# yaricom/Plastic-UNet

Hardware: AMD Instinct MI355X
Metric: training images/sec (128x128, bs=32 per GPU) (higher is better)
Workload: dtype f32; 1 GPU; C2: UNetp depth 5 base_ch 64, oja rule, 1x128x128, fwd+BCE+bwd+Adam; global_batch=32, per_gpu_batch=32, img=128, parallelism=single, step_launch=eager

## Files before the change

### plastic-unet_amd/csrc/wgrad.hip

```cpp
#include "common.h"
#include <type_traits>

#ifndef PU_NO_ILV
#define PU_NO_ILV 0
#endif
#ifndef PU_WW_ABL
#define PU_WW_ABL 0
#endif

namespace pu {

typedef float f32x4 __attribute__((ext_vector_type(4)));
typedef float f32x16 __attribute__((ext_vector_type(16)));

constexpr int WG_BM = 16;

struct WgradParams {
    int M, N, Nr, K, Kc, C, c0, c1;
    int Hi, Wi, Ho, Wo, kw, stride, pad;
    const float* P;
    const float* src0;
    const float* src1;
    int bias_mode;
    float* slab;
// ... 914 lines not shown
        sub(k, std::integral_constant<int, 1>{});
        sub(k, std::integral_constant<int, 2>{});
        sub(k, std::integral_constant<int, 3>{});
    }
    asm volatile("s_waitcnt vmcnt(0) lgkmcnt(0)" ::: "memory");

    float* slab = p.slab + (long long)z * p.Nr * p.Kcp;
    if (p.bias_mode == 1 && cx == 0) {
        wg_f32x2* red = reinterpret_cast<wg_f32x2*>(lg0);
        red[tid] = bsum;
        __syncthreads();
        if (tid < 32) {
            wg_f32x2 v = red[tid];
            for (int r = 1; r < 16; ++r) v += red[r * 32 + tid];
            slab[(long long)(ny * 64 + 2 * tid) * p.Kcp + p.K] = v[0];
            slab[(long long)(ny * 64 + 2 * tid + 1) * p.Kcp + p.K] = v[1];
        }
        __syncthreads();
    }

    const float sj1 = wj ? -1.f : 1.f;
    float* xs = reinterpret_cast<float*>(wc ? lx1 : lx0) + (wn * 2 + wj) * 24 * 64;
    const float* xrd = reinterpret_cast<const float*>(wc ? lx1 : lx0) + (wn * 2 + (1 - wj)) * 24 * 64;
    const int lr = lane & 31, lh = lane >> 5;
    const int n = ny * 64 + wn * 32 + lr;
#pragma unroll
    for (int r = 0; r < 3; ++r) {
        float mine[2][3][4], other[2][3][4];
#pragma unroll
        for (int q = 0; q < 4; ++q)
#pragma unroll
            for (int ee = 0; ee < 4; ++ee) {
                const int idx = 4 * q + ee;
                float R[2];
#pragma unroll
                for (int jj = 0; jj < 2; ++jj) {
                    const float m0 = acc[0 * 2 + jj][idx], m1 = acc[1 * 2 + jj][idx];
                    const float m2 = acc[2 * 2 + jj][idx], m3 = -acc[3 * 2 + jj][idx];
                    float v = r == 0 ? m0 + 0.5f * (m1 + m2) : r == 1 ? 0.5f * (m1 - m2) : 0.5f * (m1 + m2) + m3;
                    R[jj] = jj == 1 ? sj1 * v : v;
                }
                float P[3];
                if (wj == 0) {
                    P[0] = R[0] + 0.5f * R[1];
                    P[1] = 0.5f * R[1];
                    P[2] = 0.5f * R[1];
                } else {
                    P[0] = 0.5f * R[0];
                    P[1] = -0.5f * R[0];
                    P[2] = 0.5f * R[0] + R[1];
                }
                const bool keep = (q >> 1) == wj;
#pragma unroll
                for (int s = 0; s < 3; ++s) {
                    if (keep) mine[q & 1][s][ee] = P[s];
                    else other[q & 1][s][ee] = P[s];
                }
            }
#pragma unroll
        for (int qh = 0; qh < 2; ++qh)
#pragma unroll
            for (int s = 0; s < 3; ++s)
#pragma unroll
                for (int ee = 0; ee < 4; ++ee) xs[((qh * 3 + s) * 4 + ee) * 64 + lane] = other[qh][s][ee];
        __syncthreads();
#pragma unroll
        for (int qh = 0; qh < 2; ++qh)
#pragma unroll
            for (int s = 0; s < 3; ++s) {
                f32x4 v;
#pragma unroll
                for (int ee = 0; ee < 4; ++ee) {
                    const float o = xrd[((qh * 3 + s) * 4 + ee) * 64 + lane];
                    v[ee] = wj == 0 ? mine[qh][s][ee] + o : o + mine[qh][s][ee];
                }
                const int q = 2 * wj + qh;
                const int k = (3 * r + s) * p.C + c_lo + wc * 32 + 8 * q + 4 * lh;
                *reinterpret_cast<f32x4*>(slab + (long long)n * p.Kcp + k) = v;
            }
        __syncthreads();
    }
}

constexpr int SWS_TH = 16, SWS_TW = 64;

template <int N, bool BF16ROWS = false>
__global__ __launch_bounds__(256) void wgrad_stem_kernel(const WgradParams p) {
    constexpr int L = N / 4, PG = 256 / L;
    constexpr int HH = SWS_TH + 2, HW = SWS_TW + 2;
    constexpr int RED = PG * 10 * N;
    __shared__ __attribute__((aligned(16))) float smem[RED > HH * HW ? RED : HH * HW];
    const int tid = threadIdx.x;
    const int lane_c = tid % L, grp = tid / L;
    float acc[10][4];
#pragma unroll
    for (int k = 0; k < 10; ++k)
#pragma unroll
        for (int e = 0; e < 4; ++e) acc[k][e] = 0.f;
    const int ntiles = p.batch * p.tiles_h * p.tiles_w;
    for (int t = blockIdx.x; t < ntiles; t += gridDim.x) {
        const int txi = t % p.tiles_w;
        const int tyi = (t / p.tiles_w) % p.tiles_h;
        const int b = t / (p.tiles_w * p.tiles_h);
        const int y0 = tyi * SWS_TH - 1, x0 = txi * SWS_TW - 1;
        const long long img = (long long)b * p.Hi * p.Wi;
        __syncthreads();
        for (int e = tid; e < HH * HW; e += 256) {
            const int hy = e / HW, hx = e - hy * HW;
            const int gy = y0 + hy, gx = x0 + hx;
            smem[e] = ((unsigned)gy < (unsigned)p.Hi && (unsigned)gx < (unsigned)p.Wi)
                          ? p.src0[img + (long long)gy * p.Wi + gx] : 0.f;
        }
        __syncthreads();
        static_assert((SWS_TH * SWS_TW) % (4 * PG) == 0, "stem wgrad pass");
        for (int q0 = grp; q0 < SWS_TH * SWS_TW; q0 += 4 * PG) {
            f32x4 dzs[4];
            bool ok[4];
            int hb[4];
#pragma unroll
            for (int u = 0; u < 4; ++u) {
                const int q = q0 + u * PG;
                const int row = q / SWS_TW, col = q - row * SWS_TW;
                const int oy = tyi * SWS_TH + row, ox = txi * SWS_TW + col;
                ok[u] = oy < p.Ho && ox < p.Wo;
                hb[u] = row * HW + col;
                const long long m = ok[u] ? ((long long)b * p.Ho + oy) * p.Wo + ox : 0;
                if constexpr (BF16ROWS) {
                    typedef __bf16 bf16x4_t __attribute__((ext_vector_type(4)));
                    const bf16x4_t zb = *reinterpret_cast<const bf16x4_t*>(reinterpret_cast<const __bf16*>(p.P) + m * N + 4 * lane_c);
#pragma unroll
                    for (int e = 0; e < 4; ++e) dzs[u][e] = (float)zb[e];
                } else {
                    dzs[u] = *reinterpret_cast<const f32x4*>(p.P + m * N + 4 * lane_c);
                }
            }
#pragma unroll
            for (int u = 0; u < 4; ++u) {
                if (!ok[u]) continue;
                const f32x4 dz = dzs[u];
#pragma unroll
                for (int t9 = 0; t9 < 9; ++t9) {
                    const float a = smem[hb[u] + (t9 / 3) * HW + t9 % 3];
#pragma unroll
                    for (int e = 0; e < 4; ++e) acc[t9][e] = fmaf(a, dz[e], acc[t9][e]);
                }
#pragma unroll
                for (int e = 0; e < 4; ++e) acc[9][e] += dz[e];
            }
        }
    }
    __syncthreads();
#pragma unroll
    for (int k = 0; k < 10; ++k)
#pragma unroll
        for (int e = 0; e < 4; ++e) smem[(grp * 10 + k) * N + 4 * lane_c + e] = acc[k][e];
    __syncthreads();
    float* slab = p.slab + (long long)blockIdx.x * p.Nr * p.Kcp;
    for (int idx = tid; idx < 10 * N; idx += 256) {
        const int k = idx / N, n = idx - k * N;
        float v = 0.f;
        for (int g = 0; g < PG; ++g) v += smem[(g * 10 + k) * N + n];
        slab[(long long)n * p.Kcp + k] = v;
    }
}

template <int C, int N>
// ... 296 lines not shown
__global__ __launch_bounds__(256) void wgrad_sum_splits4_kernel(const float* __restrict__ slab, int splits,
                                                                long long total, int G, double* __restrict__ part) {
    const long long idx = 4 * (blockIdx.x * (long long)blockDim.x + threadIdx.x);
    if (idx >= total) return;
    const int g = blockIdx.y;
    const f64x4 s = sum_chains<8>(reinterpret_cast<const f32x4*>(slab + (long long)g * total + idx),
                                  (splits - g + G - 1) / G, G * (total >> 2));
    double* o = part + (long long)g * total + idx;
#pragma unroll
    for (int e = 0; e < 4; ++e) o[e] = s[e];
}

template <typename T>
__global__ __launch_bounds__(256) void wgrad_finish4_kernel(const T* __restrict__ part, int G, int Nr, int Kc, int N,
                                                            int K, int C, int kh, int kw, int bias_mode,
                                                            float* __restrict__ dw, float* __restrict__ db,
                                                            int accumulate) {
    typedef T t4 __attribute__((ext_vector_type(4)));
    const long long total = (long long)Nr * Kc;
    const long long nq = total >> 2;
    const long long q = blockIdx.x * (long long)blockDim.x + threadIdx.x;
    if (q < nq) {
        const long long idx = 4 * q;
        const int n = int(idx / Kc);
        const int k0 = int(idx - (long long)n * Kc);
        if (n >= N) return;
        const f64x4 s = sum_chains<8>(reinterpret_cast<const t4*>(part + idx), G, nq);
#pragma unroll
        for (int e = 0; e < 4; ++e) store_oihw(n, k0 + e, (float)s[e], K, C, kh, kw, bias_mode, dw, db, accumulate);
    } else if (bias_mode == 2 && q < nq + C) {
        const int c = int(q - nq);
        const int J = kh * kw * G;
        const T* bp = part + (long long)N * Kc + c;
        auto at = [&](int j) {
            const int t = j / G, gg = j - t * G;
            return (double)bp[(long long)gg * total + t * C];
        };
        double s[4] = {0.0, 0.0, 0.0, 0.0};
        int j = 0;
        for (; j + 7 < J; j += 8) {
            double v[8];
#pragma unroll
            for (int u = 0; u < 8; ++u) v[u] = at(j + u);
#pragma unroll
            for (int u = 0; u < 8; ++u) s[u & 3] += v[u];
        }
        for (; j < J; ++j) s[0] += at(j);
        const float v = (float)((s[0] + s[1]) + (s[2] + s[3]));
        db[c] = accumulate ? db[c] + v : v;
    }
}

template <typename T>
__global__ __launch_bounds__(576) void wgrad_finish_t_kernel(const T* __restrict__ part, int G, int Nr, int Kc, int K,
                                                              int C, int taps, int bias_mode, float* __restrict__ dw,
                                                              float* __restrict__ db, int accumulate) {
    __shared__ float tr[256 * 9];
    typedef T t4 __attribute__((ext_vector_type(4)));
    const long long total = (long long)Nr * Kc;
    const int n = blockIdx.y;
    const int c0 = blockIdx.x * 256;
    const int tap = threadIdx.x >> 6, cq = (threadIdx.x & 63) * 4;
    const int cn = min(256, C - c0);
    if (cq < cn) {
        const long long idx = (long long)n * Kc + tap * C + c0 + cq;
        const f64x4 s = sum_chains<4>(reinterpret_cast<const t4*>(part) + (idx >> 2), G, total >> 2);
#pragma unroll
        for (int e = 0; e < 4; ++e) tr[(cq + e) * taps + tap] = (float)s[e];
    }
    if (bias_mode == 1 && blockIdx.x == 0 && threadIdx.x == 0) {
        const float v = (float)sum_chains<4>(part + (long long)n * Kc + K, G, total);
        db[n] = accumulate ? db[n] + v : v;
    }
    __syncthreads();
    float* o = dw + ((long long)n * C + c0) * taps;
    const int run = cn * taps;
    for (int i = threadIdx.x * 4; i < run; i += blockDim.x * 4) {
        f32x4 v = {tr[i], tr[i + 1], tr[i + 2], tr[i + 3]};
        if (accumulate) v += *reinterpret_cast<const f32x4*>(o + i);
        *reinterpret_cast<f32x4*>(o + i) = v;
    }
}

struct WgradPlan {
    int BN, BK, splits, mps, Nr, Kc, Kcp, M, K, C, G, gx, gy;
    bool qvec, dma, small, halo, stem;
    bool wino = false;
    bool pw = false;
    int tiles = 0, tps = 0;
    int nt = 1;
    int tiles_w, tiles_h;
    size_t slab_bytes() const { return (size_t)splits * Nr * Kcp * sizeof(float); }
    size_t part_bytes() const { return G > 1 ? (size_t)G * Nr * Kcp * sizeof(double) : 0; }
    size_t ws_bytes() const { return ((slab_bytes() + 255) / 256) * 256 + part_bytes(); }
};

static bool stem_wgrad_ok(const pu_wgrad_args* a) {
    return a->c0 == 1 && a->c1 == 0 && (a->n == 8 || a->n == 16 || a->n == 32 || a->n == 64) && a->kh == 3 && a->kw == 3 && a->stride == 1 &&
           a->pad == 1 && a->in_h == a->out_h && a->in_w == a->out_w && a->bias_mode == 1 &&
           ((uintptr_t)a->rows & 15) == 0;
}

static bool pw_wgrad_ok(const pu_wgrad_args* a) {
    const int C = a->c0, N = a->n;
    return a->c1 == 0 && a->kh == 1 && a->kw == 1 && a->stride == 1 && a->pad == 0 && a->in_h == a->out_h &&
           a->in_w == a->out_w && a->bias_mode != 2 && (C == 3 || C == 4) && (N == 4 || N == 8 || N == 16) &&
           (((uintptr_t)a->rows & 15) == 0) && (C % 4 || ((uintptr_t)a->src0 & 15) == 0);
}

static bool small_wgrad_ok(const pu_wgrad_args* a) {
    const int C = a->c0 + a->c1;
    return (C == 1 || C == 4 || C == 8 || C == 12 || C == 16) &&
           (a->n == 4 || a->n == 8 || a->n == 16) && a->kh == 3 && a->kw == 3 && a->stride == 1 && a->pad == 1 &&
           a->in_h == a->out_h && a->in_w == a->out_w && a->bias_mode != 2 &&
           (C == 1 || (a->c0 % 4 == 0 && a->c1 % 4 == 0));
}

static void plan_groups(WgradPlan* pl) {
    const long long total = (long long)pl->Nr * pl->Kcp;
    int G = (int)ceil_div(262144LL, total);
    const int by_len = ceil_div(pl->splits, 8);
    if (G > by_len) G = by_len;
    if (G > 16) G = 16;
    pl->G = G < 1 ? 1 : G;
}

static int plan_dims(const pu_wgrad_args* a, WgradPlan* pl, const char* who) {
    const long long M = (long long)a->batch * a->out_h * a->out_w;
    PU_REQUIRE(M < (1LL << 31), "%s: too many pixels", who);
    pl->M = (int)M;
    pl->C = a->c0 + a->c1;
    pl->K = a->kh * a->kw * pl->C;
    pl->Nr = a->n + (a->bias_mode == 2 ? 1 : 0);
    pl->Kc = pl->K + (a->bias_mode == 1 ? 1 : 0);
    pl->Kcp = (pl->Kc + 3) / 4 * 4;
    return PU_OK;
}

static void plan_halo(const pu_wgrad_args* a, WgradPlan* pl) {
    pl->halo = true;
    pl->nt = a->n % 128 == 0 ? 2 : 1;
    pl->BN = 64 * pl->nt;
    pl->BK = 9 * 64;
    pl->gx = pl->C / 64;
    pl->gy = a->n / pl->BN;
    int splits = (pl->nt == 2 ? 256 : 512) / (pl->gx * pl->gy);
    const int stages = pl->M / 16;
    if (splits > stages) splits = stages;
    if (splits < 1) splits = 1;
    pl->mps = ceil_div(stages, splits) * 16;
    pl->splits = ceil_div(pl->M, pl->mps);
    plan_groups(pl);
}

static bool wino_wgrad_ok(const pu_wgrad_args* a, const WgradPlan* pl) {
    static const bool on = [] {
        const char* e = getenv("PU_WINO_WGRAD");
        return !(e && e[0] == '0');
    }();
    if (!on || a->math != 1 || !pl->qvec) return false;
    if (a->kh != 3 || a->kw != 3 || a->stride != 1 || a->pad != 1) return false;
    if (a->in_h != a->out_h || a->in_w != a->out_w || (a->out_h & 1) || (a->out_w & 1)) return false;
    if (a->c0 % 64 || a->c1 % 64 || a->n % 64 || a->bias_mode == 2) return false;
    const long long px = (long long)a->batch * a->in_h * a->in_w + a->in_w + 1;
    if (px * (a->c0 > a->c1 ? a->c0 : a->c1) * 4 >= (1LL << 31)) return false;
    if ((long long)a->batch * a->out_h * a->out_w * a->n * 4 >= (1LL << 31)) return false;
    return (((uintptr_t)a->rows | (uintptr_t)a->src0 | (uintptr_t)a->src1) & 7) == 0;
}

static int plan_wgrad(const pu_wgrad_args* a, WgradPlan* pl) {
    PU_REQUIRE(a && a->batch > 0 && a->out_h > 0 && a->out_w > 0 && a->in_h > 0 && a->in_w > 0, "pu_wgrad: bad grid");
    PU_REQUIRE(a->kh > 0 && a->kw > 0 && a->stride > 0 && a->pad >= 0, "pu_wgrad: bad taps");
    PU_REQUIRE(a->rows && a->n > 0 && a->src0 && a->c0 > 0 && (a->c1 == 0 || a->src1), "pu_wgrad: operands");
    PU_REQUIRE(a->n % 4 == 0, "pu_wgrad: n (%d) must be a multiple of 4", a->n);
    PU_REQUIRE(a->bias_mode >= 0 && a->bias_mode <= 2, "pu_wgrad: bias_mode");
    PU_REQUIRE(a->bias_mode == 0 || a->dbias, "pu_wgrad: dbias missing");
    PU_REQUIRE(a->dweight, "pu_wgrad: dweight missing");
    PU_REQUIRE(a->math >= 0 && a->math <= 2, "pu_wgrad: math %d", a->math);
    PU_REQUIRE(a->math != 2 || stem_wgrad_ok(a), "pu_wgrad: math 2 (bf16 rows) is the single-channel stem only");
    if (int st = plan_dims(a, pl, "pu_wgrad")) return st;
    const long long M = pl->M;
    pl->qvec = (a->c0 % 4 == 0) && (a->c1 % 4 == 0);
    pl->small = small_wgrad_ok(a);
    pl->stem = stem_wgrad_ok(a);
    pl->pw = pw_wgrad_ok(a);
    pl->halo = false;
    if (pl->qvec) {
        PU_REQUIRE(((uintptr_t)a->src0 & 15) == 0 && ((uintptr_t)a->src1 & 15) == 0, "pu_wgrad: sources must be 16-byte aligned");
    }
    PU_REQUIRE(((uintptr_t)a->rows & 15) == 0, "pu_wgrad: rows must be 16-byte aligned");
    pl->dma = pl->qvec;
    if (pl->pw) {
        pl->splits = (int)(M / 256 < 1024 ? (M + 255) / 256 : 1024);
        pl->mps = (int)ceil_div(M, (long long)pl->splits);
        pl->splits = (int)ceil_div(M, (long long)pl->mps);
        pl->BN = a->n; pl->BK = pl->K; pl->gx = pl->gy = 1; pl->dma = false;
        pl->tiles_w = pl->tiles_h = 0;
        plan_groups(pl);
        return PU_OK;
    }
    if (pl->small || pl->stem) {
        pl->tiles_w = ceil_div(a->out_w, pl->stem ? SWS_TW : SW_TW);
        pl->tiles_h = ceil_div(a->out_h, pl->stem ? SWS_TH : SW_TH);
        const long long ntiles = (long long)a->batch * pl->tiles_w * pl->tiles_h;
        pl->splits = (int)(ntiles < 1024 ? ntiles : 1024);
        pl->BN = a->n; pl->BK = pl->K; pl->gx = pl->gy = 1; pl->mps = 0; pl->dma = false;
        plan_groups(pl);
        return PU_OK;
    }
    const int ext_n = pl->dma ? a->n : pl->Nr;
    const int ext_k = pl->dma ? pl->K : pl->Kc;
    int occ;
    if (ext_k <= 64) { pl->BN = 64; pl->BK = 64; occ = pl->dma ? 6 : 7; }
    else if (ext_n <= 64 && !pl->dma) { pl->BN = 64; pl->BK = 256; occ = 3; }
    else if (ext_n <= 32 && a->math == 1) { pl->BN = 32; pl->BK = 128; occ = 4; }
    else if (ext_n <= 64) {
        const bool b192 = ceil_div(ext_k, 192) * 192 < ceil_div(ext_k, 128) * 128;
        pl->BN = 64; pl->BK = b192 ? 192 : 128; occ = b192 ? 3 : 4;
    }
    else { pl->BN = 128; pl->BK = 128; occ = pl->dma ? 3 : 4; }
    if (a->math == 1 && pl->dma && pl->BN == 128 &&
        ceil_div(ext_k, 256) * 256 <= ceil_div(ext_k, 128) * 128) {
        pl->BK = 256;
        occ = 2;
    }
    pl->halo = false;
    if (wino_wgrad_ok(a, pl)) {
        pl->wino = true;
        pl->BN = 64;
        pl->BK = 9 * 64;
        pl->gx = pl->C / 64;
        pl->gy = a->n / 64;
        pl->tiles = a->batch * (a->out_h / 2) * (a->out_w / 2);
        const int stages = ceil_div(pl->tiles, 16);
        int splits = 256 / (pl->gx * pl->gy);
        if (splits > stages) splits = stages;
        if (splits < 1) splits = 1;
        pl->tps = ceil_div(stages, splits) * 16;
        pl->splits = ceil_div(pl->tiles, pl->tps);
        pl->mps = pl->tps * 4;
        plan_groups(pl);
        return PU_OK;
    }
    if (a->math == 1 && pl->dma && a->kh == 3 && a->kw == 3 && a->stride == 1 && a->pad == 1 &&
        a->in_h == a->out_h && a->in_w == a->out_w && a->out_w % 16 == 0 && a->c0 % 64 == 0 && a->c1 % 64 == 0 &&
        a->n % 64 == 0 && a->bias_mode != 2 && (long long)a->batch * a->in_h * a->in_w * (pl->C) < (1LL << 31)) {
        plan_halo(a, pl);
        return PU_OK;
    }
    pl->gx = ceil_div(ext_k, pl->BK);
    pl->gy = ceil_div(ext_n, pl->BN);
    const int tiles = pl->gx * pl->gy;
    const int slots = 256 * occ;
    int splits = slots / tiles;
    int max_splits = ceil_div(M, 256);
    if (splits > max_splits) splits = max_splits;
    if (splits < 1) splits = 1;
    int mps = ceil_div(ceil_div(M, splits), WG_BM) * WG_BM;
    pl->mps = mps;
    pl->splits = ceil_div(M, mps);
    plan_groups(pl);
    return PU_OK;
}

typedef __bf16 wbf16x8 __attribute__((ext_vector_type(8)));
__device__ __attribute__((aligned(16))) __bf16 g_wg_zero_b16[8];

constexpr int WB_ROWS = 32;
constexpr int WB_W = 128;


struct WgradBf16Params {
    int M, N, K, Kcp, Nr, C, c0, c1;
    int Hi, Wi, Ho, Wo, kw, stride, pad;
    const __bf16* P;
    const __bf16* src0;
    const __bf16* src1;
    int bias_mode;
    float* slab;
    int mps, gx, gy;
    FastDiv dWo, dHo, dC, dKw;
};

__global__ __launch_bounds__(256) void wgrad_bf16_kernel(const WgradBf16Params p) {
    constexpr int NBUF = 3;
    constexpr int LD = WB_ROWS * WB_W * 2 / 1024 / 4;
    constexpr int G = 2 * LD;
    constexpr int IMG = WB_ROWS * WB_W;
    constexpr int STAGE = 2 * IMG;
    __shared__ __attribute__((aligned(16))) __bf16 lds[NBUF * STAGE];

    const int tid = threadIdx.x;
    const int lane = tid & 63;
    const int wave = __builtin_amdgcn_readfirstlane(tid >> 6);
    const int wn = wave & 1, wk = wave >> 1;
    const int lr = lane & 31, lh = lane >> 5;
    const int tile = xcd_remap(blockIdx.x, gridDim.x);
    const int tx = tile % p.gx;
    const int tyz = tile / p.gx;
    const int ty = tyz % p.gy;
    const int tz = tyz / p.gy;
    const int n_blk = ty * WB_W;
    const int k_blk = tx * WB_W;
    const int m_begin = tz * p.mps;
    const int m_end = min(p.M, m_begin + p.mps);

    const int lrow = lane >> 4;
    int p_col[LD], q_r[LD], q_s[LD], q_cs[LD];
    const __bf16* q_ptr[LD];
// ... 283 lines not shown
        asm volatile("s_waitcnt lgkmcnt(0)" ::: "memory");
        __builtin_amdgcn_s_barrier();
        asm volatile("" ::: "memory");
    }
    int g = 0;
    for (; g + 1 < NG; g += 2) {
        group(g, std::integral_constant<int, 0>{});
        group(g + 1, std::integral_constant<int, 1>{});
    }
    if (g < NG) group(g, std::integral_constant<int, 0>{});

    float* slab = p.slab + (long long)tz * p.Nr * p.Kcp;
    if (bias_blk) {
        f32x4* red = reinterpret_cast<f32x4*>(lds);
        red[tid] = bsum;
        __syncthreads();
        if (tid < 16 * NT) {
            f32x4 v = red[tid];
            for (int r = 1; r < 16; ++r) v += red[r * 16 * NT + tid];
#pragma unroll
            for (int e = 0; e < 4; ++e) slab[(long long)(ty * 64 * NT + tid * 4 + e) * p.Kcp + p.K] = v[e];
        }
    }
    const int lr = lane & 31, lh = lane >> 5;
    const int n = ty * 64 * NT + nt * 64 + nj * 32 + lr;
#pragma unroll
    for (int t9 = 0; t9 < 9; ++t9) {
#pragma unroll
        for (int q = 0; q < 4; ++q) {
            const int k = t9 * p.C + c_lo + ci * 32 + 8 * q + 4 * lh;
            f32x4 v;
#pragma unroll
            for (int e = 0; e < 4; ++e) v[e] = acc[t9][4 * q + e];
            *reinterpret_cast<f32x4*>(slab + (long long)n * p.Kcp + k) = v;
        }
    }
}

constexpr int WR_E = 16, WR_S = 64;
__global__ __launch_bounds__(256) void wgrad_reduce_wide_kernel(const float* __restrict__ slab, int splits,
                                                                 long long total, int N, int Kcp, int K, int C,
                                                                 int kh, int kw, int bias_mode, float* __restrict__ dw,
                                                                 float* __restrict__ db, int accumulate) {
    __shared__ double part[WR_S][WR_E];
    const int quad = threadIdx.x & 3, sl = threadIdx.x >> 2;
    const long long idx0 = (long long)blockIdx.x * WR_E + 4 * quad;
    f64x4 a = {};
    if (idx0 < total)
        a = sum_chains<4>(reinterpret_cast<const f32x4*>(slab + (long long)sl * total + idx0),
                          (splits - sl + WR_S - 1) / WR_S, WR_S * (total >> 2));
#pragma unroll
    for (int e = 0; e < 4; ++e) part[sl][4 * quad + e] = a[e];
    __syncthreads();
    if (threadIdx.x >= WR_E) return;
    const long long idx = (long long)blockIdx.x * WR_E + threadIdx.x;
    if (idx >= total) return;
    double sum = 0.0;
    for (int l = 0; l < WR_S; ++l) sum += part[l][threadIdx.x];
    const int n = (int)(idx / Kcp), k = (int)(idx - (long long)n * Kcp);
    if (n >= N) return;
    store_oihw(n, k, (float)sum, K, C, kh, kw, bias_mode, dw, db, accumulate);
}

template <typename T>
static void launch_finisher(bool transposed, const T* part, int count, const WgradPlan& pl, const pu_wgrad_args* a,
                            hipStream_t s) {
    const int taps = a->kh * a->kw;
    if (transposed) {
        hipLaunchKernelGGL(wgrad_finish_t_kernel<T>, dim3((unsigned)ceil_div(pl.C, 256), (unsigned)a->n),
                           dim3((unsigned)(64 * taps)), 0, s, part, count, pl.Nr, pl.Kcp, pl.K, pl.C, taps, a->bias_mode,
                           a->dweight, a->dbias, a->accumulate);
        return;
    }
    const long long threads = (long long)pl.Nr * pl.Kcp / 4 + (a->bias_mode == 2 ? pl.C : 0);
    hipLaunchKernelGGL(wgrad_finish4_kernel<T>, dim3((unsigned)((threads + 255) / 256)), dim3(256), 0, s, part, count,
                       pl.Nr, pl.Kcp, a->n, pl.K, pl.C, a->kh, a->kw, a->bias_mode, a->dweight, a->dbias, a->accumulate);
}

constexpr long long WR_WIDE_MAX = 16384;

static int wgrad_reduce(const WgradPlan& pl, const pu_wgrad_args* a, void* workspace, hipStream_t s) {
    const long long total = (long long)pl.Nr * pl.Kcp;
    const float* slab = (const float*)workspace;
    if ((pl.small || pl.stem || pl.pw || (!pl.wino && total <= WR_WIDE_MAX)) && a->bias_mode != 2) {
        hipLaunchKernelGGL(wgrad_reduce_wide_kernel, dim3((unsigned)ceil_div(total, (long long)WR_E)), dim3(256), 0, s,
                           slab, pl.splits, total, a->n, pl.Kcp, pl.K, pl.C, a->kh, a->kw, a->bias_mode, a->dweight,
                           a->dbias, a->accumulate);
        return check_launch("pu_wgrad (reduce)");
    }
    const bool transposed = a->bias_mode != 2 && a->kh * a->kw <= 9 && pl.C % 4 == 0 && ((uintptr_t)a->dweight & 15) == 0;
    if (pl.G > 1) {
        double* part = (double*)((char*)workspace + ((pl.slab_bytes() + 255) / 256) * 256);
        hipLaunchKernelGGL(wgrad_sum_splits4_kernel, dim3((unsigned)((total / 4 + 255) / 256), pl.G), dim3(256), 0, s,
                           slab, pl.splits, total, pl.G, part);
        launch_finisher(transposed, (const double*)part, pl.G, pl, a, s);
    } else {
        launch_finisher(transposed, slab, pl.splits, pl, a, s);
    }
    return check_launch("pu_wgrad (reduce)");
}

static int plan_wgrad_bf16(const pu_wgrad_args* a, WgradPlan* pl) {
    PU_REQUIRE(a && a->batch > 0 && a->out_h > 0 && a->out_w > 0 && a->in_h > 0 && a->in_w > 0, "pu_wgrad_bf16: bad grid");
    PU_REQUIRE(a->kh > 0 && a->kw > 0 && a->stride > 0 && a->pad >= 0, "pu_wgrad_bf16: bad taps");
    PU_REQUIRE(a->rows && a->n > 0 && a->src0 && a->c0 > 0 && (a->c1 == 0 || a->src1), "pu_wgrad_bf16: operands");
    PU_REQUIRE(a->n % 8 == 0 && a->c0 % 8 == 0 && a->c1 % 8 == 0,
               "pu_wgrad_bf16: n (%d) and channel counts (%d, %d) must be multiples of 8", a->n, a->c0, a->c1);
    PU_REQUIRE(a->bias_mode >= 0 && a->bias_mode <= 2 && (a->bias_mode == 0 || a->dbias) && a->dweight, "pu_wgrad_bf16: outputs");
    PU_REQUIRE((((uintptr_t)a->rows | (uintptr_t)a->src0 | (uintptr_t)a->src1) & 15) == 0, "pu_wgrad_bf16: 16-byte alignment");
    if (int st = plan_dims(a, pl, "pu_wgrad_bf16")) return st;
    const long long M = pl->M;
    pl->qvec = true; pl->dma = true; pl->small = false; pl->stem = false;
    pl->halo = false;
    if (a->kh == 3 && a->kw == 3 && a->stride == 1 && a->pad == 1 && a->in_h == a->out_h &&
        a->in_w == a->out_w && a->out_w % 16 == 0 && a->c0 % 64 == 0 && a->c1 % 64 == 0 && a->n % 64 == 0 &&
        a->bias_mode != 2 && M * pl->C < (1LL << 31)) {
        plan_halo(a, pl);
        return PU_OK;
    }
    pl->BN = WB_W; pl->BK = WB_W;
    pl->gx = ceil_div(pl->K, WB_W);
    pl->gy = ceil_div(a->n, WB_W);
    const int tiles = pl->gx * pl->gy;
    int splits = 768 / tiles;
    const int max_splits = ceil_div(M, 512);
    if (splits > max_splits) splits = max_splits;
    if (splits < 1) splits = 1;
    pl->mps = ceil_div(ceil_div(M, splits), WB_ROWS) * WB_ROWS;
    pl->splits = ceil_div(M, pl->mps);
    plan_groups(pl);
    return PU_OK;
}

}

using namespace pu;

extern "C" size_t pu_wgrad_workspace_bytes(const pu_wgrad_args* a) {
    WgradPlan pl;
    if (plan_wgrad(a, &pl) != PU_OK) return 0;
    return pl.ws_bytes();
}

extern "C" int pu_wgrad_tile(const pu_wgrad_args* a, int* bn, int* bk, int* qvec, int* splits) {
    WgradPlan pl;
    int st = plan_wgrad(a, &pl);
    if (st != PU_OK) return st;
    if (bn) *bn = pl.BN;
    if (bk) *bk = pl.BK;
    if (qvec) *qvec = pl.pw ? 6 : pl.wino ? 5 : pl.stem ? 4 : pl.small ? 2 : pl.halo ? 3 : (pl.qvec ? 1 : 0);
    if (splits) *splits = pl.splits;
    return PU_OK;
}

extern "C" int pu_wgrad(const pu_wgrad_args* a, void* workspace, size_t ws_bytes, void* stream) {
    return pu_wgrad_phase(a, workspace, ws_bytes, 3, stream);
}

extern "C" int pu_wgrad_phase(const pu_wgrad_args* a, void* workspace, size_t ws_bytes, int phase, void* stream) {
    PU_REQUIRE(phase >= 1 && phase <= 3, "pu_wgrad_phase: phase %d", phase);
    WgradPlan pl;
    int st = plan_wgrad(a, &pl);
    if (st != PU_OK) return st;
    const size_t need = pl.ws_bytes();
    if (!workspace || ws_bytes < need)
        return fail(PU_ERR_WORKSPACE, "pu_wgrad: workspace %zu < %zu bytes", ws_bytes, need);

    WgradParams p;
    p.M = pl.M; p.N = a->n; p.Nr = pl.Nr; p.K = pl.K; p.Kc = pl.Kc; p.Kcp = pl.Kcp; p.C = pl.C; p.c0 = a->c0; p.c1 = a->c1;
    p.Hi = a->in_h; p.Wi = a->in_w; p.Ho = a->out_h; p.Wo = a->out_w;
    p.kw = a->kw; p.stride = a->stride; p.pad = a->pad;
    p.P = a->rows; p.src0 = a->src0; p.src1 = a->src1; p.bias_mode = a->bias_mode;
    p.slab = (float*)workspace; p.mps = pl.mps;
    p.dWo = make_fastdiv(a->out_w); p.dHo = make_fastdiv(a->out_h);
    p.dC = make_fastdiv(pl.C); p.dKw = make_fastdiv(a->kw);

    hipStream_t s = as_stream(stream);
    p.gx = pl.gx;
    p.gy = pl.gy;
    p.batch = a->batch; p.tiles_w = pl.tiles_w; p.tiles_h = pl.tiles_h;
    if (pl.stem && (phase & 1) && a->math == 2) {
        if (a->n == 64) hipLaunchKernelGGL((wgrad_stem_kernel<64, true>), dim3(pl.splits), dim3(256), 0, s, p);
        else if (a->n == 32) hipLaunchKernelGGL((wgrad_stem_kernel<32, true>), dim3(pl.splits), dim3(256), 0, s, p);
        else if (a->n == 16) hipLaunchKernelGGL((wgrad_stem_kernel<16, true>), dim3(pl.splits), dim3(256), 0, s, p);
        else hipLaunchKernelGGL((wgrad_stem_kernel<8, true>), dim3(pl.splits), dim3(256), 0, s, p);
        st = check_launch("pu_wgrad (stem, bf16 rows)");
        if (st != PU_OK) return st;
        phase &= ~1;
    }
    if (pl.stem && (phase & 1)) {
        if (a->n == 64) hipLaunchKernelGGL(wgrad_stem_kernel<64>, dim3(pl.splits), dim3(256), 0, s, p);
        else if (a->n == 32) hipLaunchKernelGGL(wgrad_stem_kernel<32>, dim3(pl.splits), dim3(256), 0, s, p);
        else if (a->n == 16) hipLaunchKernelGGL(wgrad_stem_kernel<16>, dim3(pl.splits), dim3(256), 0, s, p);
        else hipLaunchKernelGGL(wgrad_stem_kernel<8>, dim3(pl.splits), dim3(256), 0, s, p);
        st = check_launch("pu_wgrad (stem)");
        if (st != PU_OK) return st;
        phase &= ~1;
    }
    if (pl.pw && (phase & 1)) {
        const int C = pl.C, N = a->n;
        const dim3 sg(pl.splits);
#define PU_PW(C_, N_) if (C == C_ && N == N_) hipLaunchKernelGGL((wgrad_pw_kernel<C_, N_>), sg, dim3(256), 0, s, p)
        PU_PW(3, 4); else PU_PW(3, 8); else PU_PW(3, 16); else PU_PW(4, 4); else PU_PW(4, 8); else PU_PW(4, 16);
#undef PU_PW
        st = check_launch("pu_wgrad (pointwise)");
        if (st != PU_OK) return st;
        phase &= ~1;
    }
    if (pl.small && (phase & 1)) {
        const int C = pl.C, N = a->n;
        const dim3 sg(pl.splits);
#define PU_SW(C_, N_) if (C == C_ && N == N_) hipLaunchKernelGGL((wgrad_small_kernel<C_, N_>), sg, dim3(256), 0, s, p)
        PU_SW(1, 4); else PU_SW(1, 8); else PU_SW(1, 16); else PU_SW(4, 4); else PU_SW(4, 8); else PU_SW(4, 16);
        else PU_SW(8, 4); else PU_SW(8, 8); else PU_SW(8, 16); else PU_SW(12, 4); else PU_SW(12, 8);
        else PU_SW(12, 16); else PU_SW(16, 4); else PU_SW(16, 8); else PU_SW(16, 16);
#undef PU_SW
        st = check_launch("pu_wgrad (small-channel)");
        if (st != PU_OK) return st;
        phase &= ~1;
    }
    dim3 grid(p.gx * p.gy * pl.splits);
    const bool fq = a->stride == 1 && a->in_h == a->out_h && a->in_w == a->out_w && a->out_w >= 4;
    if (phase & 1) {
#define PU_WG_DMA(BN_, BK_, WN_, WK_)                                                                    \
    do {                                                                                                     \
        if (a->math == 1 && fq) hipLaunchKernelGGL((wgrad_dma_kernel<BN_, BK_, WN_, WK_, 3, true, 4, true>), grid, dim3(256), 0, s, p); \
        else if (a->math == 1) hipLaunchKernelGGL((wgrad_dma_kernel<BN_, BK_, WN_, WK_, 3, true>), grid, dim3(256), 0, s, p); \
        else hipLaunchKernelGGL((wgrad_dma_kernel<BN_, BK_, WN_, WK_, 3, false>), grid, dim3(256), 0, s, p); \
    } while (0)
#define PU_WG_REG(BN_, BK_, WN_, WK_, Q_) hipLaunchKernelGGL((wgrad_kernel<BN_, BK_, WN_, WK_, Q_>), grid, dim3(256), 0, s, p)
        if (pl.wino) {
            WinoWgradParams ww;
            ww.p = p;
            ww.tiles = pl.tiles;
            ww.tps = pl.tps;
            ww.dTw = make_fastdiv(a->out_w / 2);
            ww.dTh = make_fastdiv(a->out_h / 2);
            const long long px = (long long)a->batch * a->in_h * a->in_w + a->in_w + 1;
            ww.x0_bytes = (unsigned)(px * a->c0 * 4);
            ww.x1_bytes = (unsigned)(px * a->c1 * 4);
            ww.p_bytes = (unsigned)((long long)pl.M * a->n * 4);
            hipLaunchKernelGGL(wgrad_wino_x6_kernel, grid, dim3(512), 0, s, ww);
        } else if (pl.halo) {
            if (pl.nt == 2) hipLaunchKernelGGL(wgrad_halo_x6_kernel<2>, grid, dim3(512), 0, s, p);
            else hipLaunchKernelGGL(wgrad_halo_x6_kernel<1>, grid, dim3(256), 0, s, p);
        } else if (pl.dma) {
            if (pl.BK == 64) PU_WG_DMA(64, 64, 2, 2);
            else if (pl.BN == 64 && pl.BK == 128) PU_WG_DMA(64, 128, 2, 2);
            else if (pl.BN == 32) PU_WG_DMA(32, 128, 1, 4);
            else if (pl.BK == 192) PU_WG_DMA(64, 192, 2, 2);
            else if (pl.BK == 256 && fq) hipLaunchKernelGGL((wgrad_dma_kernel<128, 256, 2, 2, 3, true, 4, true>), grid, dim3(256), 0, s, p);
            else if (pl.BK == 256) hipLaunchKernelGGL((wgrad_dma_kernel<128, 256, 2, 2, 3, true>), grid, dim3(256), 0, s, p);
            else PU_WG_DMA(128, 128, 2, 2);
        } else if (pl.qvec) {
            if (pl.BK == 64) PU_WG_REG(64, 64, 2, 2, true);
            else if (pl.BK == 256) PU_WG_REG(64, 256, 1, 4, true);
            else PU_WG_REG(128, 128, 2, 2, true);
        } else {
            if (pl.BK == 64) PU_WG_REG(64, 64, 2, 2, false);
            else if (pl.BK == 256) PU_WG_REG(64, 256, 1, 4, false);
            else PU_WG_REG(128, 128, 2, 2, false);
        }
#undef PU_WG_DMA
#undef PU_WG_REG
        st = check_launch("pu_wgrad (gemm)");
        if (st != PU_OK) return st;
    }
    if (!(phase & 2)) return PU_OK;
    return wgrad_reduce(pl, a, workspace, s);
}

extern "C" size_t pu_wgrad_bf16_workspace_bytes(const pu_wgrad_args* a) {
    WgradPlan pl;
    if (plan_wgrad_bf16(a, &pl) != PU_OK) return 0;
    return pl.ws_bytes();
}

extern "C" int pu_wgrad_bf16_phase(const pu_wgrad_args* a, void* workspace, size_t ws_bytes, int phase, void* stream) {
    PU_REQUIRE(phase >= 1 && phase <= 3, "pu_wgrad_bf16_phase: phase %d", phase);
    WgradPlan pl;
    int st = plan_wgrad_bf16(a, &pl);
    if (st != PU_OK) return st;
    const size_t need = pl.ws_bytes();
    if (!workspace || ws_bytes < need)
        return fail(PU_ERR_WORKSPACE, "pu_wgrad_bf16: workspace %zu < %zu bytes", ws_bytes, need);
    hipStream_t s = as_stream(stream);
    if (phase & 1) {
        WgradBf16Params p;
        p.M = pl.M; p.N = a->n; p.K = pl.K; p.Kcp = pl.Kcp; p.Nr = pl.Nr; p.C = pl.C; p.c0 = a->c0; p.c1 = a->c1;
        p.Hi = a->in_h; p.Wi = a->in_w; p.Ho = a->out_h; p.Wo = a->out_w;
        p.kw = a->kw; p.stride = a->stride; p.pad = a->pad;
        p.P = (const __bf16*)a->rows; p.src0 = (const __bf16*)a->src0; p.src1 = (const __bf16*)a->src1;
        p.bias_mode = a->bias_mode;
        p.slab = (float*)workspace; p.mps = pl.mps; p.gx = pl.gx; p.gy = pl.gy;
        p.dWo = make_fastdiv(a->out_w); p.dHo = make_fastdiv(a->out_h);
        p.dC = make_fastdiv(pl.C); p.dKw = make_fastdiv(a->kw);
        if (pl.halo && pl.nt == 2) hipLaunchKernelGGL(wgrad_halo_bf16_kernel<2>, dim3(pl.gx * pl.gy * pl.splits), dim3(512), 0, s, p);
        else if (pl.halo) hipLaunchKernelGGL(wgrad_halo_bf16_kernel<1>, dim3(pl.gx * pl.gy * pl.splits), dim3(256), 0, s, p);
        else hipLaunchKernelGGL(wgrad_bf16_kernel, dim3(pl.gx * pl.gy * pl.splits), dim3(256), 0, s, p);
        st = check_launch("pu_wgrad_bf16 (gemm)");
        if (st != PU_OK) return st;
    }
    if (!(phase & 2)) return PU_OK;
    return wgrad_reduce(pl, a, workspace, s);
}

extern "C" int pu_wgrad_bf16_tile(const pu_wgrad_args* a, int* bn, int* bk, int* halo, int* splits) {
    WgradPlan pl;
    int st = plan_wgrad_bf16(a, &pl);
    if (st != PU_OK) return st;
    if (bn) *bn = pl.BN;
    if (bk) *bk = pl.BK;
    if (halo) *halo = pl.halo ? 1 : 0;
    if (splits) *splits = pl.splits;
    return PU_OK;
}

extern "C" int pu_wgrad_bf16(const pu_wgrad_args* a, void* workspace, size_t ws_bytes, void* stream) {
    return pu_wgrad_bf16_phase(a, workspace, ws_bytes, 3, stream);
}
```

Measured before the change: 4812 images/s.

## Add column-split Winograd weight-gradient kernel with fused column-transform finisher

Adds a new Winograd F(2,3) weight-gradient path for 3x3 convolutions whose channel counts are multiples of 128 and which have enough output tiles. The work is split across four column-transform blocks (J) with 128x128 output tiles and 3-split bf16 MFMA emulation of fp32. A dedicated finisher kernel folds the four per-column partial slabs back into 3x3 weights, reducing in double precision. This is meant to improve reuse and MFMA utilisation on the large inner layers compared with the 64-wide Winograd kernel. In exchange it adds a larger LDS footprint, a different reduction order, and a new launch-path branch.

```diff
diff --git a/plastic-unet_amd/csrc/wgrad.hip b/plastic-unet_amd/csrc/wgrad.hip
--- a/plastic-unet_amd/csrc/wgrad.hip
+++ b/plastic-unet_amd/csrc/wgrad.hip
@@ -1020,6 +1020,265 @@
     }
 }
 
+constexpr int WWR_IMG = 16 * 256;
+constexpr int WWR_SLOT = 2 * 3 * WWR_IMG;
+__device__ __forceinline__ int wwr_off(int row, int col) {
+    return row * 256 + 16 * ((col >> 3) ^ wb_sw(row)) + 2 * (col & 7);
+}
+
+__global__ __launch_bounds__(512) void wgrad_wino_cols_x6_kernel(const WinoWgradParams w) {
+#pragma clang fp contract(off)
+    const WgradParams& p = w.p;
+    __shared__ __attribute__((aligned(16))) char lx0[WWR_SLOT];
+    __shared__ __attribute__((aligned(16))) char lx1[WWR_SLOT];
+    __shared__ __attribute__((aligned(16))) char lg0[WWR_SLOT];
+    __shared__ __attribute__((aligned(16))) char lg1[WWR_SLOT];
+
+    const int tid = threadIdx.x;
+    const int lane = tid & 63;
+    const int wave = __builtin_amdgcn_readfirstlane(tid >> 6);
+    const int wc = wave & 1, wn = wave >> 1;
+    const int blk = xcd_remap(blockIdx.x, gridDim.x);
+    const int J = blk & 3;
+    const int cx = (blk >> 2) % p.gx;
+    const int rest = (blk >> 2) / p.gx;
+    const int ny = rest % p.gy;
+    const int z = rest / p.gy;
+    const int t_begin = z * w.tps;
+    const int t_end = min(w.tiles, t_begin + w.tps);
+    const int S = (t_end - t_begin + 15) >> 4;
+    const int xca = J == 0 ? 0 : J == 2 ? 2 : 1, xcb = J == 3 ? 3 : J == 2 ? 1 : 2;
+    const float sxf = J == 1 ? 1.f : -1.f;
+    const int gca = J == 3 ? 1 : 0;
+    const bool gtwo = J == 1 || J == 2;
+    const float sgf = J == 2 ? -1.f : 1.f;
+    const wg_f32x2 sx2 = {sxf, sxf}, sg2 = {sgf, sgf};
+
+    const int pt = tid >> 5, cq = tid & 31;
+    const int c_lo = cx * 128;
+    const bool first = c_lo < p.c0;
+    const int cs = first ? p.c0 : p.c1;
+    const int shift = p.Wi + 1;
+    const __amdgpu_buffer_rsrc_t xr = ww_rsrc((first ? p.src0 : p.src1) - (long long)shift * cs,
+                                              first ? w.x0_bytes : w.x1_bytes);
+    const __amdgpu_buffer_rsrc_t gr = ww_rsrc(p.P, w.p_bytes);
+    const unsigned pixb = (unsigned)cs * 4u;
+    const unsigned xco = (unsigned)((first ? c_lo : c_lo - p.c0) + 4 * cq) * 4u;
+    const unsigned gco = (unsigned)(ny * 128 + 4 * cq) * 4u;
+    const unsigned gpix = (unsigned)p.N * 4u;
+    const int st_off = wwr_off(pt, 4 * cq);
+
+    wg_f32x2 da[4][2], db[4][2], ea[2][2], eb[2][2];
+    auto load_stage = [&](int k) {
+        const int m = t_begin + 16 * k + pt;
+        const bool mv = m < t_end;
+        int ty = 0, tx = 0, b = 0;
+        if (mv) {
+            const int t2 = fdiv(m, w.dTw);
+            tx = m - t2 * (p.Wo >> 1);
+            b = fdiv(t2, w.dTh);
+            ty = t2 - b * (p.Ho >> 1);
+        }
+        const int y0 = 2 * ty - 1, x0 = 2 * tx - 1;
+        const unsigned base = (unsigned)(((b * p.Hi + y0) * p.Wi + x0 + shift) * cs) * 4u + xco;
+        const bool cva = mv && (xca != 0 || x0 >= 0), cvb = mv && (xcb != 3 || x0 + 3 < p.Wi);
+#pragma unroll
+        for (int r = 0; r < 4; ++r) {
+            const bool rv = (unsigned)(y0 + r) < (unsigned)p.Hi;
+            const unsigned oa = cva && rv ? base + (unsigned)xca * pixb : LEAN_OOB;
+            const unsigned ob = cvb && rv ? base + (unsigned)xcb * pixb : LEAN_OOB;
+            const unsigned so = __builtin_amdgcn_readfirstlane((unsigned)(r * p.Wi) * pixb);
+            const f32x4 a4 = __builtin_bit_cast(f32x4, __builtin_amdgcn_raw_buffer_load_b128(xr, oa, so, 0));
+            const f32x4 b4 = __builtin_bit_cast(f32x4, __builtin_amdgcn_raw_buffer_load_b128(xr, ob, so, 0));
+            da[r][0] = wg_f32x2{a4[0], a4[1]}; da[r][1] = wg_f32x2{a4[2], a4[3]};
+            db[r][0] = wg_f32x2{b4[0], b4[1]}; db[r][1] = wg_f32x2{b4[2], b4[3]};
+        }
+        const unsigned gbase = (unsigned)((b * p.Ho + 2 * ty) * p.Wo + 2 * tx) * gpix + gco;
+        const unsigned ga_ = mv ? gbase + (unsigned)gca * gpix : LEAN_OOB;
+        const unsigned gb_ = mv && gtwo ? gbase + gpix : LEAN_OOB;
+#pragma unroll
+        for (int a = 0; a < 2; ++a) {
+            const unsigned so = __builtin_amdgcn_readfirstlane((unsigned)(a * p.Wo) * gpix);
+            const f32x4 a4 = __builtin_bit_cast(f32x4, __builtin_amdgcn_raw_buffer_load_b128(gr, ga_, so, 0));
+            const f32x4 b4 = __builtin_bit_cast(f32x4, __builtin_amdgcn_raw_buffer_load_b128(gr, gb_, so, 0));
+            ea[a][0] = wg_f32x2{a4[0], a4[1]}; ea[a][1] = wg_f32x2{a4[2], a4[3]};
+            eb[a][0] = wg_f32x2{b4[0], b4[1]}; eb[a][1] = wg_f32x2{b4[2], b4[3]};
+        }
+    };
+    auto put = [&](const wg_f32x2 (&v)[2], char* b) {
+        unsigned h0, m0, l0, h1, m1, l1;
+        ww_split(v[0], h0, m0, l0);
+        ww_split(v[1], h1, m1, l1);
+        typedef unsigned wu32x2 __attribute__((ext_vector_type(2)));
+        *reinterpret_cast<wu32x2*>(b) = wu32x2{h0, h1};
+        *reinterpret_cast<wu32x2*>(b + WWR_IMG) = wu32x2{m0, m1};
+        *reinterpret_cast<wu32x2*>(b + 2 * WWR_IMG) = wu32x2{l0, l1};
+    };
+    wg_f32x2 hd[2][2], he[2][2];
+    wg_f32x2 bsum[2] = {{0.f, 0.f}, {0.f, 0.f}};
+    auto form_a = [&](char* sx, char* sg) {
+        wg_f32x2 dv0[2], dv1[2], ev0[2], ev1[2];
+#pragma unroll
+        for (int hf = 0; hf < 2; ++hf) {
+            const wg_f32x2 ta[4] = {da[0][hf] - da[2][hf], da[1][hf] + da[2][hf], da[2][hf] - da[1][hf], da[1][hf] - da[3][hf]};
+            const wg_f32x2 tb[4] = {db[0][hf] - db[2][hf], db[1][hf] + db[2][hf], db[2][hf] - db[1][hf], db[1][hf] - db[3][hf]};
+            const wg_f32x2 ua[4] = {ea[0][hf], ea[0][hf] + ea[1][hf], ea[0][hf] - ea[1][hf], ea[1][hf]};
+            const wg_f32x2 ub[4] = {eb[0][hf], eb[0][hf] + eb[1][hf], eb[0][hf] - eb[1][hf], eb[1][hf]};
+            dv0[hf] = __builtin_elementwise_fma(tb[0], sx2, ta[0]);
+            dv1[hf] = __builtin_elementwise_fma(tb[1], sx2, ta[1]);
+            hd[0][hf] = __builtin_elementwise_fma(tb[2], sx2, ta[2]);
+            hd[1][hf] = __builtin_elementwise_fma(tb[3], sx2, ta[3]);
+            ev0[hf] = __builtin_elementwise_fma(ub[0], sg2, ua[0]);
+            ev1[hf] = __builtin_elementwise_fma(ub[1], sg2, ua[1]);
+            he[0][hf] = __builtin_elementwise_fma(ub[2], sg2, ua[2]);
+            he[1][hf] = __builtin_elementwise_fma(ub[3], sg2, ua[3]);
+            bsum[hf] += ea[0][hf] + eb[0][hf];
+            bsum[hf] += ea[1][hf] + eb[1][hf];
+        }
+        put(dv0, sx + st_off);
+        put(ev0, sg + st_off);
+        put(dv1, sx + 3 * WWR_IMG + st_off);
+        put(ev1, sg + 3 * WWR_IMG + st_off);
+    };
+    auto form_b = [&](char* sx, char* sg) {
+        put(hd[0], sx + st_off);
+        put(he[0], sg + st_off);
+        put(hd[1], sx + 3 * WWR_IMG + st_off);
+        put(he[1], sg + 3 * WWR_IMG + st_off);
+    };
+
+    const int grp = lane >> 4, gq = (lane >> 2) & 3, gp = lane & 3;
+    const int rsub = 8 * (grp >> 1) + gq;
+    const int ccol = 16 * (grp & 1) + 4 * gp;
+    int xo[2][2], go[2];
+#pragma unroll
+    for (int hh = 0; hh < 2; ++hh) {
+        xo[0][hh] = wwr_off(rsub + 4 * hh, wc * 64 + ccol);
+        xo[1][hh] = wwr_off(rsub + 4 * hh, wc * 64 + 32 + ccol);
+        go[hh] = wwr_off(rsub + 4 * hh, wn * 32 + ccol);
+    }
+    auto tr2 = [&](const char* b, int o0, int o1) {
+        const wi16x4 a0 = __builtin_amdgcn_ds_read_tr16_b64_v4i16((lds_i16x4_t*)(b + o0));
+        const wi16x4 a1 = __builtin_amdgcn_ds_read_tr16_b64_v4i16((lds_i16x4_t*)(b + o1));
+        typedef short wi16x8 __attribute__((ext_vector_type(8)));
+        const wi16x8 av = {a0[0], a0[1], a0[2], a0[3], a1[0], a1[1], a1[2], a1[3]};
+        return __builtin_bit_cast(wg_bf16x8, av);
+    };
+    f32x16 acc[8];
+#pragma unroll
+    for (int x = 0; x < 8; ++x)
+#pragma unroll
+        for (int r = 0; r < 16; ++r) acc[x][r] = 0.f;
+    auto mma = [&](auto j_c, const char* sx, const char* sg, int jj) {
+        constexpr int j = decltype(j_c)::value;
+        const char* gb = sg + jj * 3 * WWR_IMG;
+        const wg_bf16x8 ph = tr2(gb, go[0], go[1]), pm = tr2(gb + WWR_IMG, go[0], go[1]),
+                        pl = tr2(gb + 2 * WWR_IMG, go[0], go[1]);
+#pragma unroll
+        for (int f = 0; f < 2; ++f) {
+            const char* xb = sx + jj * 3 * WWR_IMG;
+            const wg_bf16x8 qh = tr2(xb, xo[f][0], xo[f][1]), qm = tr2(xb + WWR_IMG, xo[f][0], xo[f][1]),
+                            ql = tr2(xb + 2 * WWR_IMG, xo[f][0], xo[f][1]);
+            f32x16 c = acc[4 * f + j];
+            c = __builtin_amdgcn_mfma_f32_32x32x16_bf16(qm, pm, c, 0, 0, 0);
+            c = __builtin_amdgcn_mfma_f32_32x32x16_bf16(ql, ph, c, 0, 0, 0);
+            c = __builtin_amdgcn_mfma_f32_32x32x16_bf16(qh, pl, c, 0, 0, 0);
+            c = __builtin_amdgcn_mfma_f32_32x32x16_bf16(qm, ph, c, 0, 0, 0);
+            c = __builtin_amdgcn_mfma_f32_32x32x16_bf16(qh, pm, c, 0, 0, 0);
+            c = __builtin_amdgcn_mfma_f32_32x32x16_bf16(qh, ph, c, 0, 0, 0);
+            acc[4 * f + j] = c;
+        }
+    };
+
+    auto sub = [&](int k, auto h_c) {
+        constexpr int h = decltype(h_c)::value;
+        char* sx = h ? lx1 : lx0;
+        char* sg = h ? lg1 : lg0;
+        char* nx = h ? lx0 : lx1;
+        char* ng = h ? lg0 : lg1;
+        mma(std::integral_constant<int, 2 * h>{}, sx, sg, 0);
+        if constexpr (h == 0) {
+            form_b(nx, ng);
+        } else {
+            form_a(nx, ng);
+            load_stage(k + 2);
+        }
+        mma(std::integral_constant<int, 2 * h + 1>{}, sx, sg, 1);
+#if !PU_NO_ILV
+        __builtin_amdgcn_sched_group_barrier(0x100, 12, 0);
+#pragma unroll
+        for (int q = 0; q < 24; ++q) {
+            __builtin_amdgcn_sched_group_barrier(0x008, 1, 0);
+            if (q == 0 || q == 12) __builtin_amdgcn_sched_group_barrier(0x100, 6, 0);
+            if (q == 6) __builtin_amdgcn_sched_group_barrier(0x100, 12, 0);
+            __builtin_amdgcn_sched_group_barrier(0x002, 5, 0);
+            if (q & 1) __builtin_amdgcn_sched_group_barrier(0x200, 1, 0);
+        }
+#endif
+        asm volatile("s_waitcnt lgkmcnt(0)" ::: "memory");
+        __builtin_amdgcn_s_barrier();
+        asm volatile("" ::: "memory");
+    };
+
+    load_stage(0);
+    form_a(lx0, lg0);
+    load_stage(1);
+    asm volatile("s_waitcnt lgkmcnt(0)" ::: "memory");
+    __builtin_amdgcn_s_barrier();
+    asm volatile("" ::: "memory");
+    for (int k = 0; k < S; ++k) {
+        sub(k, std::integral_constant<int, 0>{});
+        sub(k, std::integral_constant<int, 1>{});
+    }
+    asm volatile("s_waitcnt vmcnt(0) lgkmcnt(0)" ::: "memory");
+
+    float* slab = p.slab + (long long)(4 * z + J) * p.Nr * p.Kcp;
+    if (p.bias_mode == 1 && cx == 0 && J == 1) {
+        wg_f32x2* red = reinterpret_cast<wg_f32x2*>(lg0);
+        red[2 * tid] = bsum[0];
+        red[2 * tid + 1] = bsum[1];
+        __syncthreads();
+        if (tid < 64) {
+            wg_f32x2 v = red[tid];
+            for (int r = 1; r < 16; ++r) v += red[r * 64 + tid];
+            slab[(long long)(ny * 128 + 2 * tid) * p.Kcp + p.K] = v[0];
+            slab[(long long)(ny * 128 + 2 * tid + 1) * p.Kcp + p.K] = v[1];
+        }
+        __syncthreads();
+    }
+
+    constexpr int TP = 68;
+    const float kap = J == 3 ? -1.f : 1.f;
+    float* wt = reinterpret_cast<float*>((wave >> 1) == 0 ? lx0 : (wave >> 1) == 1 ? lx1 : (wave >> 1) == 2 ? lg0 : lg1) +
+                (wave & 1) * (32 * TP);
+    const int ln = lane & 31, lh = lane >> 5;
+    const int rr = lane >> 4, rc = (lane & 15) * 4;
+    float* obase = slab + (long long)(ny * 128 + wn * 32 + rr) * p.Kcp + c_lo + wc * 64 + rc;
+#pragma unroll
+    for (int r = 0; r < 3; ++r) {
+#pragma unroll
+        for (int f = 0; f < 2; ++f)
+#pragma unroll
+            for (int q = 0; q < 4; ++q) {
+                f32x4 t;
+#pragma unroll
+                for (int ee = 0; ee < 4; ++ee) {
+                    const int idx = 4 * q + ee;
+                    const float m0 = acc[4 * f][idx], m1 = acc[4 * f + 1][idx];
+                    const float m2 = acc[4 * f + 2][idx], m3 = -acc[4 * f + 3][idx];
+                    const float hs = 0.5f * (m1 + m2);
+                    t[ee] = kap * (r == 0 ? m0 + hs : r == 1 ? 0.5f * (m1 - m2) : hs + m3);
+                }
+                *reinterpret_cast<f32x4*>(wt + ln * TP + 32 * f + 8 * q + 4 * lh) = t;
+            }
+#pragma unroll
+        for (int it = 0; it < 8; ++it) {
+            const f32x4 v = *reinterpret_cast<const f32x4*>(wt + (rr + 4 * it) * TP + rc);
+            *reinterpret_cast<f32x4*>(obase + (long long)(4 * it) * p.Kcp + r * p.C) = v;
+        }
+    }
+}
+
 constexpr int SWS_TH = 16, SWS_TW = 64;
 
 template <int N, bool BF16ROWS = false>
@@ -1482,10 +1741,123 @@
     }
 }
 
+template <int NV, typename F>
+__device__ __forceinline__ void chain_values(int count, F&& v, f64x4 (&out)[NV]) {
+    f64x4 s[NV][4] = {};
+    int i = 0;
+    for (; i + 4 <= count; i += 4) {
+        f32x4 q[4][NV];
+#pragma unroll
+        for (int u = 0; u < 4; ++u) v(i + u, q[u]);
+#pragma unroll
+        for (int u = 0; u < 4; ++u)
+#pragma unroll
+            for (int e = 0; e < NV; ++e) s[e][u] += widen(q[u][e]);
+    }
+    for (; i < count; ++i) {
+        f32x4 q[NV];
+        v(i, q);
+#pragma unroll
+        for (int e = 0; e < NV; ++e) s[e][0] += widen(q[e]);
+    }
+#pragma unroll
+    for (int e = 0; e < NV; ++e) out[e] = (s[e][0] + s[e][1]) + (s[e][2] + s[e][3]);
+}
+
+__global__ __launch_bounds__(384) void wgrad_finish_cols_kernel(const float* __restrict__ slab, int zs, int G, int Nr,
+                                                                 int Kcp, int C, int bias_mode, float* __restrict__ dw,
+                                                                 float* __restrict__ db, int accumulate, int vec) {
+#pragma clang fp contract(off)
+    __shared__ float tr[256 * 9];
+    __shared__ double pp[2][9][256];
+    __shared__ double pb[2];
+    const long long total = (long long)Nr * Kcp;
+    const int n = blockIdx.y;
+    const int c0 = blockIdx.x * 256;
+    const int g = threadIdx.x / 192, t = threadIdx.x - g * 192;
+    const int r = t >> 6, cq = (t & 63) * 4;
+    const int cn = min(256, C - c0);
+    const int count = (zs - g + G - 1) / G;
+    f64x4 acc[3];
+    if (cq < cn) {
+        const float* base = slab + (long long)n * Kcp + r * C + c0 + cq;
+        chain_values<3>(count, [&](int i, f32x4 (&q)[3]) {
+            const float* pz = base + (long long)(4 * (g + i * G)) * total;
+            const f32x4 R0 = *reinterpret_cast<const f32x4*>(pz), R1 = *reinterpret_cast<const f32x4*>(pz + total);
+            const f32x4 R2 = *reinterpret_cast<const f32x4*>(pz + 2 * total), R3 = *reinterpret_cast<const f32x4*>(pz + 3 * total);
+            const f32x4 h1 = 0.5f * R1, h2 = 0.5f * R2;
+            q[0] = (R0 + h1) + h2;
+            q[1] = h1 + (-0.5f * R2);
+            q[2] = h1 + (h2 + R3);
+        }, acc);
+        if (G > 1) {
+#pragma unroll
+            for (int s = 0; s < 3; ++s)
+#pragma unroll
+                for (int e = 0; e < 4; ++e) pp[g][3 * r + s][cq + e] = acc[s][e];
+        }
+    }
+    double bacc = 0.0;
+    const bool bias_thread = bias_mode == 1 && blockIdx.x == 0 && t == 0;
+    if (bias_thread) {
+        const float* bp = slab + total + (long long)n * Kcp + 3 * C;
+        double s4[4] = {0.0, 0.0, 0.0, 0.0};
+        int i = 0;
+        for (; i + 4 <= count; i += 4)
+#pragma unroll
+            for (int u = 0; u < 4; ++u) s4[u] += (double)bp[(long long)(4 * (g + (i + u) * G)) * total];
+        for (; i < count; ++i) s4[0] += (double)bp[(long long)(4 * (g + i * G)) * total];
+        bacc = (s4[0] + s4[1]) + (s4[2] + s4[3]);
+        if (G > 1) pb[g] = bacc;
+    }
+    __syncthreads();
+    if (g == 0) {
+        if (cq < cn) {
+#pragma unroll
+            for (int s = 0; s < 3; ++s)
+#pragma unroll
+                for (int e = 0; e < 4; ++e) {
+                    double v = acc[s][e];
+                    if (G > 1) {
+                        double c4[4] = {0.0, 0.0, 0.0, 0.0};
+                        c4[0] += pp[0][3 * r + s][cq + e];
+                        c4[0] += pp[1][3 * r + s][cq + e];
+                        v = (c4[0] + c4[1]) + (c4[2] + c4[3]);
+                    }
+                    tr[(cq + e) * 9 + 3 * r + s] = (float)v;
+                }
+        }
+        if (bias_thread) {
+            double v = bacc;
+            if (G > 1) {
+                double c4[4] = {0.0, 0.0, 0.0, 0.0};
+                c4[0] += pb[0];
+                c4[0] += pb[1];
+                v = (c4[0] + c4[1]) + (c4[2] + c4[3]);
+            }
+            db[n] = accumulate ? db[n] + (float)v : (float)v;
+        }
+    }
+    __syncthreads();
+    float* o = dw + ((long long)n * C + c0) * 9;
+    const int run = cn * 9;
+    if (vec) {
+        for (int i = threadIdx.x * 4; i < run; i += blockDim.x * 4) {
+            f32x4 v = {tr[i], tr[i + 1], tr[i + 2], tr[i + 3]};
+            if (accumulate) v += *reinterpret_cast<const f32x4*>(o + i);
+            *reinterpret_cast<f32x4*>(o + i) = v;
+        }
+    } else {
+        for (int i = threadIdx.x; i < run; i += blockDim.x) o[i] = accumulate ? o[i] + tr[i] : tr[i];
+    }
+}
+
 struct WgradPlan {
     int BN, BK, splits, mps, Nr, Kc, Kcp, M, K, C, G, gx, gy;
     bool qvec, dma, small, halo, stem;
     bool wino = false;
+    bool cols = false;
+    int Gfin = 1;
     bool pw = false;
     int tiles = 0, tps = 0;
     int nt = 1;
@@ -1552,6 +1924,8 @@
     pl->splits = ceil_div(pl->M, pl->mps);
     plan_groups(pl);
 }
+
+constexpr int WWR_MIN_TILES = 512;
 
 static bool wino_wgrad_ok(const pu_wgrad_args* a, const WgradPlan* pl) {
     static const bool on = [] {
@@ -1625,6 +1999,33 @@
         occ = 2;
     }
     pl->halo = false;
+    if (wino_wgrad_ok(a, pl) && a->c0 % 128 == 0 && a->c1 % 128 == 0 && a->n % 128 == 0 &&
+        a->batch * (a->out_h / 2) * (a->out_w / 2) >= WWR_MIN_TILES) {
+        pl->wino = pl->cols = true;
+        pl->BN = 128;
+        pl->BK = 3 * 128;
+        pl->gx = pl->C / 128;
+        pl->gy = a->n / 128;
+        pl->tiles = a->batch * (a->out_h / 2) * (a->out_w / 2);
+        const int stages = ceil_div(pl->tiles, 16);
+        int zs = 256 / (4 * pl->gx * pl->gy);
+        if (zs > stages) zs = stages;
+        if (zs < 1) zs = 1;
+        pl->tps = ceil_div(stages, zs) * 16;
+        pl->splits = 4 * ceil_div(pl->tiles, pl->tps);
+        pl->mps = pl->tps * 4;
+        pl->Kc = 3 * pl->C + (a->bias_mode == 1 ? 1 : 0);
+        pl->Kcp = (pl->Kc + 3) / 4 * 4;
+        {
+            WgradPlan q = *pl;
+            q.splits = pl->splits / 4;
+            q.Kcp = (9 * pl->C + (a->bias_mode == 1 ? 1 : 0) + 3) / 4 * 4;
+            plan_groups(&q);
+            pl->Gfin = q.G;
+        }
+        pl->G = 1;
+        return PU_OK;
+    }
     if (wino_wgrad_ok(a, pl)) {
         pl->wino = true;
         pl->BN = 64;
@@ -2074,6 +2475,13 @@
 static int wgrad_reduce(const WgradPlan& pl, const pu_wgrad_args* a, void* workspace, hipStream_t s) {
     const long long total = (long long)pl.Nr * pl.Kcp;
     const float* slab = (const float*)workspace;
+    if (pl.cols) {
+        const dim3 fg((unsigned)ceil_div(pl.C, 256), (unsigned)a->n);
+        const int vec = ((uintptr_t)a->dweight & 15) == 0;
+        hipLaunchKernelGGL(wgrad_finish_cols_kernel, fg, dim3(192 * pl.Gfin), 0, s, slab, pl.splits / 4, pl.Gfin, pl.Nr,
+                           pl.Kcp, pl.C, a->bias_mode, a->dweight, a->dbias, a->accumulate, vec);
+        return check_launch("pu_wgrad (reduce)");
+    }
     if ((pl.small || pl.stem || pl.pw || (!pl.wino && total <= WR_WIDE_MAX)) && a->bias_mode != 2) {
         hipLaunchKernelGGL(wgrad_reduce_wide_kernel, dim3((unsigned)ceil_div(total, (long long)WR_E)), dim3(256), 0, s,
                            slab, pl.splits, total, a->n, pl.Kcp, pl.K, pl.C, a->kh, a->kw, a->bias_mode, a->dweight,
@@ -2232,7 +2640,12 @@
             ww.x0_bytes = (unsigned)(px * a->c0 * 4);
             ww.x1_bytes = (unsigned)(px * a->c1 * 4);
             ww.p_bytes = (unsigned)((long long)pl.M * a->n * 4);
-            hipLaunchKernelGGL(wgrad_wino_x6_kernel, grid, dim3(512), 0, s, ww);
+            if (pl.cols) {
+                ww.p.K = 3 * pl.C;
+                hipLaunchKernelGGL(wgrad_wino_cols_x6_kernel, grid, dim3(512), 0, s, ww);
+            } else {
+                hipLaunchKernelGGL(wgrad_wino_x6_kernel, grid, dim3(512), 0, s, ww);
+            }
         } else if (pl.halo) {
             if (pl.nt == 2) hipLaunchKernelGGL(wgrad_halo_x6_kernel<2>, grid, dim3(512), 0, s, p);
             else hipLaunchKernelGGL(wgrad_halo_x6_kernel<1>, grid, dim3(256), 0, s, p);
```

Result: faster. 4909 images/s (median of 6 runs) (+2.0%).
